# thangvubk/SoftGroup

Hardware: AMD Instinct MI355X
Metric: scans/sec ScanNet-v2-like inference (softgroup_scannet.yaml, full forward_test) (higher is better)
Workload: dtype f32

## Files before the change

softgroup_amd/csrc/common.h:

```cpp
#pragma once
#include <hip/hip_runtime.h>
#include <stdint.h>
#include <stdio.h>

#include "../../include/softgroup_hip.h"

namespace sg {

constexpr int kWave = 64;

void set_error(const char *fmt, ...);
int32_t *pinned_words();

inline hipStream_t as_stream(sg_stream_t s) { return reinterpret_cast<hipStream_t>(s); }

inline int check_launch(const char *what) {
  hipError_t e = hipGetLastError();
  if (e != hipSuccess) {
    set_error("%s: %s", what, hipGetErrorString(e));
    return SG_ERR_LAUNCH;
  }
  return SG_OK;
}

// ... 55 lines not shown
  v += dpp_or_zero<0x142, 0xa>(v);
  v += dpp_or_zero<0x143, 0xc>(v);
  return v;
}
__device__ __forceinline__ int wave_sum(int v) {
  return __builtin_amdgcn_readlane(wave_incl_scan(v), 63);
}
__device__ __forceinline__ int wave_max(int v) {
#pragma unroll
  for (int o = 32; o > 0; o >>= 1) v = max(v, __shfl_xor(v, o, 64));
  return v;
}

constexpr int kFillMax = 16;
struct FillList {
  uint32_t *p[kFillMax];
  size_t words[kFillMax];
  uint32_t pattern[kFillMax];
  int n = 0;
  void add(void *ptr, size_t bytes, int byte) {
    if (bytes == 0 || ptr == nullptr || n >= kFillMax) return;
    p[n] = static_cast<uint32_t *>(ptr);
    words[n] = bytes / 4;
    pattern[n] = 0x01010101u * static_cast<uint32_t>(byte & 0xff);
    ++n;
  }
};
static __global__ void __launch_bounds__(256) fill_many_kernel(FillList f) {
  const int r = blockIdx.y;
  uint32_t *p = f.p[r];
  const size_t w = f.words[r];
  const uint32_t v = f.pattern[r];
  const size_t head = (16 - (reinterpret_cast<uintptr_t>(p) & 15)) / 4 % 4;
  const size_t h = head < w ? head : w;
  const size_t quads = (w - h) / 4;
  uint4 *q = reinterpret_cast<uint4 *>(p + h);
  const uint4 vv = make_uint4(v, v, v, v);
  for (size_t i = blockIdx.x * 256ull + threadIdx.x; i < quads; i += gridDim.x * 256ull) q[i] = vv;
  if (blockIdx.x == 0) {
    if (threadIdx.x < h) p[threadIdx.x] = v;
    const size_t t0 = h + quads * 4;
    if (threadIdx.x < w - t0) p[t0 + threadIdx.x] = v;
  }
}
inline void fill_many(const FillList &f, hipStream_t stream) {
  if (f.n == 0) return;
  size_t mx = 0;
  for (int i = 0; i < f.n; ++i) mx = f.words[i] > mx ? f.words[i] : mx;
  const int gx = grid_for(static_cast<int64_t>(mx / 4 + 1), 256, 1024);
  fill_many_kernel<<<dim3(gx, f.n), 256, 0, stream>>>(f);
}

extern thread_local int t_conv_arith;
void conv_chain_begin(hipStream_t stream);
bool conv_chain_recording();
int conv_chain_end();
void conv_chain_abort();
int conv_chain_concat(const float *a, const float *b, int64_t rows, int ca, int cb, const float *scale,
                      const float *shift, float *out, float *out_act);
int conv_chain_bn_relu(const float *x, const float *scale, const float *shift, int64_t rows, int c, float *out);
int conv_chain_check_abort(const char *who);
int conv_gather_rows(const void *in, int num_in_rows, const int32_t *nbr, int M_out, int K, int Cin, int Cout,
                     const float *w_k8, const float *post_scale, const float *post_shift, const void *residual,
                     const float *act_scale, const float *act_shift, void *out_act, const int32_t *order,
                     const uint32_t *tile_mask, const int32_t *nbr_tiles, void *out, void *ws, size_t ws_bytes,
                     sg_stream_t stream, int in16, int out16, int res16);
int spconv_wgrad_layout(const void *in, int in_bf16, const void *g_out, int g_bf16, const int32_t *nbr_t, int M_out,
                        int K, int Cin, int Cout, float *dw, int out_oki, void *ws, size_t ws_bytes,
                        sg_stream_t stream);
struct PackJob {
  const float *w;
  float *out;
  int cout, kvol, cin, mode;
};
int spconv_pack_weights(const PackJob *jobs, int n, sg_stream_t stream);
size_t octree_stash_bytes(int n);
int octree_ballquery_count_stash(const float *points, const float *boxes, const int32_t *pt_inds,
                                 const int32_t *pt_start_len, int n, float radius, int32_t *start_len, int32_t *stash,
                                 hipStream_t stream);
int octree_ballquery_fill_stash(const float *points, const float *boxes, const int32_t *pt_inds,
                                const int32_t *pt_start_len, int n, float radius, const int32_t *start_len,
                                const int32_t *stash, int32_t *idx, hipStream_t stream);
void conv_release_stream(int dev, hipStream_t stream);
void unet_release_stream(int dev, hipStream_t stream);
void scan_release_stream(int dev, hipStream_t stream);
void bfs_release_stream(int dev, hipStream_t stream);
constexpr int kBfsGiantMin = 16384;
struct BfsDefer {
  bool deferred = false;
  hipStream_t side = nullptr;
};
void bfs_emit_defer(BfsDefer *d);
int bfs_emit_join(const BfsDefer &d, hipStream_t stream);
int bfs_label_max_kept(const void *ws);
int bfs_count_kept_members(const void *ws, size_t ws_bytes, int n, int64_t n_edges, const int32_t *l2p, int n_pts,
                           const float *thr_dev, int32_t *out, hipStream_t stream);

}
```

softgroup_amd/csrc/spconv_conv.hip:

```cpp
#include <stdlib.h>

#include <atomic>
#include <cstdio>
#include <map>
#include <mutex>
#include <utility>
#include <vector>

#include "common.h"

namespace sg {

typedef float f32x16 __attribute__((ext_vector_type(16)));
typedef float f4 __attribute__((ext_vector_type(4)));
typedef float f2 __attribute__((ext_vector_type(2)));
typedef __bf16 bf16x8 __attribute__((ext_vector_type(8)));
typedef __bf16 bf16x2 __attribute__((ext_vector_type(2)));

__device__ __forceinline__ void split3(const float (&x)[8], bf16x8 &h, bf16x8 &m, bf16x8 &l) {
#pragma unroll
  for (int j = 0; j < 4; ++j) {
    const f2 v = {x[2 * j], x[2 * j + 1]};
    const bf16x2 hh = __builtin_convertvector(v, bf16x2);
    const f2 r = v - __builtin_convertvector(hh, f2);
// ... 18 lines not shown
__device__ __forceinline__ uint16_t bf16_rne(float x) {
  const uint32_t u = __builtin_bit_cast(uint32_t, x);
  return static_cast<uint16_t>((u + 0x7fffu + ((u >> 16) & 1u)) >> 16);
}
__device__ __forceinline__ float bf16_f32(uint16_t b) {
  return __builtin_bit_cast(float, static_cast<uint32_t>(b) << 16);
}

#ifndef SG_WHATIF
#define SG_WHATIF 0
#endif

constexpr int kTileRows = 32;
constexpr int kWavesPerWg = 4;
constexpr int kCk = 16;
constexpr int kMaxK = 27;
constexpr int kTicketStride = 32;
constexpr unsigned kOob = 0x80000000u;

__device__ __forceinline__ void lds_dma_b128(const void *gsrc, unsigned lds_dst) {
  unsigned keep;
  asm volatile("s_mov_b32 %0, m0\n\ts_mov_b32 m0, %2\n\ts_nop 0\n\tglobal_load_lds_dwordx4 %1, off\n\t"
               "s_mov_b32 m0, %0"
               : "=&s"(keep) : "v"(gsrc), "s"(lds_dst) : "memory");
}
__device__ __forceinline__ void lds_dma_b32(const void *gsrc, unsigned lds_dst) {
  unsigned keep;
  asm volatile("s_mov_b32 %0, m0\n\ts_mov_b32 m0, %2\n\ts_nop 0\n\tglobal_load_lds_dword %1, off\n\t"
               "s_mov_b32 m0, %0"
               : "=&s"(keep) : "v"(gsrc), "s"(lds_dst) : "memory");
}

struct ConvArgs {
  const float *in;
  const int32_t *nbr;
  const float *w;
  const float *post_scale;
  const float *post_shift;
  const float *residual;
  const float *act_scale;
  const float *act_shift;
  float *out_act;
  const int32_t *order;
  const uint32_t *tile_mask;
  const int32_t *nbr_tiles;
  float *out;
  int M_out, K, Cin, Cout;
  int col_units;
  int blocks_per_unit;
  int ksplit;
  int k_per_split;
  int num_units;
  unsigned magic_upt, magic_cu, magic_nsl;
  int out16, res16;
  int dyn_rounds;
  unsigned *queue;
  unsigned long long *trace;
  unsigned *done;
  float *out_final;
};

template <int NBW, bool VEC>
__global__ void __launch_bounds__(256) gather_conv_tile_kernel(ConvArgs p) {
  extern __shared__ __attribute__((aligned(16))) char smem_raw[];
  const int wave = threadIdx.x >> 6, lane = threadIdx.x & 63;
  int32_t *nbr_lds = reinterpret_cast<int32_t *>(smem_raw) + wave * kTileRows * kMaxK;
  const int cin_pad = (p.Cin + kCk - 1) / kCk * kCk;
  const int c8 = (p.Cin + 7) / 8;

  const int num_tiles = (p.M_out + kTileRows - 1) / kTileRows;
  const int units_per_tile = p.col_units * p.ksplit;
  const long long unit = static_cast<long long>(blockIdx.x) * kWavesPerWg + wave;
  const bool valid = unit < static_cast<long long>(num_tiles) * units_per_tile;
  int tile = valid ? static_cast<int>(unit / units_per_tile) : 0;
  const int sub = valid ? static_cast<int>(unit % units_per_tile) : 0;
  const int cu = sub % p.col_units, ks = sub / p.col_units;
  const int nb0 = cu * p.blocks_per_unit;
  const int nbw = valid ? min(p.blocks_per_unit, (p.Cout + 31) / 32 - nb0) : 0;
  const int k_lo = ks * p.k_per_split, k_hi = min(p.K, k_lo + p.k_per_split);

  const int arow = lane & 31, ahalf = lane >> 5;
  int my_row = -1;
  if (valid) {
    const int pos = tile * kTileRows + arow;
    if (p.order) my_row = p.order[pos];
    else if (pos < p.M_out) my_row = pos;
  }
  if (valid) {
    for (int e = lane; e < kTileRows * p.K; e += 64) {
      const int r = e / p.K, k = e - r * p.K;
      const int row = __shfl(my_row, r, 64);
      nbr_lds[r * kMaxK + k] = row >= 0 ? p.nbr[static_cast<long long>(row) * p.K + k] : -1;
    }
  }
  __syncthreads();
  if (!valid) return;

  uint32_t mask = p.tile_mask ? p.tile_mask[tile] : 0xffffffffu;
  mask &= (k_hi >= 32 ? 0xffffffffu : ((1u << k_hi) - 1u)) & ~((1u << k_lo) - 1u);

  f32x16 acc[NBW];
#pragma unroll
  for (int n = 0; n < NBW; ++n)
#pragma unroll
    for (int r = 0; r < 16; ++r) acc[n][r] = 0.f;

// ... 256 lines not shown
      }
      const int s_w = planes_at + (k * c8 + s * 4) * p.Cout * 16;
#pragma unroll
      for (int n = 0; n < NBW; ++n)
#pragma unroll
        for (int sl = 0; sl < 2; ++sl)
#pragma unroll
          for (int pl = 0; pl < NPL; ++pl) {
            if ((SG_WHATIF & 1) && pl > 0) { S.b[n][sl * NPL + pl] = S.b[n][sl * NPL]; continue; }
            S.b[n][sl * NPL + pl] = __builtin_bit_cast(f4, __builtin_amdgcn_raw_buffer_load_b128(
                                                             rs_w, c.v_w + n * 512,
                                                             s_w + sl * (2 * p.Cout * 16) + pl * plane_bytes, 0));
          }
      return;
    }
    const int src = c.meta[nbr_base + k];
    const unsigned v_a = src >= 0 ? static_cast<unsigned>(src * p.Cin + ahalf * HC) * 4u : kOob;
    const int s_a = s * (CK * 4);
#pragma unroll
    for (int q = 0; q < NQ; ++q)
      S.a[q] = __builtin_bit_cast(f4, __builtin_amdgcn_raw_buffer_load_b128(rs_in, v_a + q * 16, s_a, AUX));
    if constexpr (SPLIT) {
      const int s_w = planes_at + (k * c8 + s * 2) * p.Cout * 16;
#pragma unroll
      for (int n = 0; n < NBW; ++n)
#pragma unroll
        for (int pl = 0; pl < NPL; ++pl)
          S.b[n][pl] = __builtin_bit_cast(f4, __builtin_amdgcn_raw_buffer_load_b128(
                                                  rs_w, c.v_w + n * 512, s_w + pl * plane_bytes, 0));
    } else {
      const int s_w = (k * c8 + s * (CK / 8)) * p.Cout * 32;
#pragma unroll
      for (int n = 0; n < NBW; ++n)
#pragma unroll
        for (int q = 0; q < NQ; ++q)
          S.b[n][q] = __builtin_bit_cast(f4, __builtin_amdgcn_raw_buffer_load_b128(
                                                 rs_w, c.v_w + n * 1024 + (q & 1) * 16,
                                                 s_w + (q >> 1) * (p.Cout * 32), 0));
    }
  };

  auto advance = [&](const Ctx &c, int &k, int &s) {
    if (++s == n_slices) {
      s = 0;
      const uint32_t rest = c.wg_mask & ~((2u << k) - 1u);
      k = rest ? __builtin_ctz(rest) : k;
    }
  };

  auto setup = [&](const Unit &d, int buf, Ctx &c) {
    c.ks = d.ks;
    c.pair = d.tile * p.col_units + d.cu;
    c.meta = meta_lds + buf * kMetaInts;
    uint32_t m = static_cast<uint32_t>(c.meta[kMaskAt]);
    if (!final_out) {
      const int k_lo = d.ks * p.k_per_split, k_hi = min(p.K, k_lo + p.k_per_split);
      m &= ((1u << k_hi) - 1u) & ~((1u << k_lo) - 1u);
    }
    m = __builtin_amdgcn_readfirstlane(m);
    c.wg_mask = m;
    c.col = d.cu * (32 * NBW) + arow;
    c.col_ok = c.col < p.Cout;
    const int colc = min(c.col, p.Cout - 1);
    c.v_w = SPLIT ? (ahalf * p.Cout + colc) * 16 : (ahalf * (HC / 8) * p.Cout + colc) * 32;
    const int items = __builtin_popcount(m) * n_slices;
    const int per = (items + WV - 1) >> WV_SHIFT;
    const int begin = min(items, wave * per);
    c.rem = min(items, begin + per) - begin;
    int rank = udiv(begin, p.magic_nsl);
    c.s = begin - rank * n_slices;
    uint32_t mm = m;
    for (; rank > 0; --rank) mm &= mm - 1u;
    c.k = mm ? __builtin_ctz(mm) : 0;
    load(c, c.k, c.s, S[0]);
    c.kp = c.k;
    c.sp = c.s;
#pragma unroll
    for (int i = 1; i < DEPTH - 1; ++i) {
      if (i < c.rem) advance(c, c.kp, c.sp);
      load(c, c.kp, c.sp, S[i]);
    }
    int row4[RR];
#pragma unroll
    for (int rr = 0; rr < RR; ++rr) {
      const int reg = wave * RR + rr;
      row4[rr] = c.meta[kRowsAt + (reg & 3) + 8 * (reg >> 2) + 4 * ahalf];
    }
#pragma unroll
    for (int rr = 0; rr < RR; ++rr) {
      const unsigned off = (row4[rr] >= 0 && c.col_ok)
                               ? static_cast<unsigned>(row4[rr] * p.Cout + c.col) * 4u : kOob;
      c.o_off[rr] = off;
#pragma unroll
      for (int n = 0; n < NBW; ++n)
        resv[n][rr] = ld_row(rs_res, off, n, res16);
    }
#pragma unroll
    for (int n = 0; n < NBW; ++n) {
      c.ps[n] = c.pb[n] = c.as[n] = c.ab[n] = 0.f;
      if (post) {
        c.ps[n] = p.post_scale[colc + 32 * n];
        c.pb[n] = p.post_shift[colc + 32 * n];
      }
      if (act) {
        c.as[n] = p.act_scale[colc + 32 * n];
        c.ab[n] = p.act_shift[colc + 32 * n];
      }
    }
  };

  f32x16 acc[NBW];
  auto compute = [&](Slice &S) {
    if constexpr (R16) {
#pragma unroll
      for (int q = 0; q < 4; ++q) {
        const int r = 8 * q + (lane >> 3);
        tr_lds[r * 8 + ((lane & 7) ^ ((r >> 1) & 7))] = S.a[q];
      }
      f4 fr[4];
#pragma unroll
      for (int sl = 0; sl < 4; ++sl) fr[sl] = tr_lds[arow * 8 + ((sl * 2 + ahalf) ^ ((arow >> 1) & 7))];
// ... 204 lines not shown

    float v[NBW][RR], va[NBW][RR];
    unsigned o_off[RR];
    {
      float part[NBW][RR][WV];
#pragma unroll
      for (int n = 0; n < NBW; ++n)
#pragma unroll
        for (int rr = 0; rr < RR; ++rr) {
          const int reg = wave * RR + rr;
#pragma unroll
          for (int w = 0; w < WV; ++w) part[n][rr][w] = red[((w * NBW + n) * 16 + reg) * 64 + lane];
        }
#pragma unroll
      for (int rr = 0; rr < RR; ++rr) {
#pragma unroll
        for (int n = 0; n < NBW; ++n) {
          float t = part[n][rr][0];
#pragma unroll
          for (int w = 1; w < WV; ++w) t += part[n][rr][w];
          t += resv[n][rr];
          if (post) t = fmaxf(fmaf(t, c.ps[n], c.pb[n]), 0.f);
          v[n][rr] = t;
          va[n][rr] = fmaxf(fmaf(t, c.as[n], c.ab[n]), 0.f);
        }
        o_off[rr] = c.o_off[rr];
      }
    }
    const unsigned o_base = final_out ? 0u : static_cast<unsigned>(c.ks) * out_bytes;
    const int rem_done = c.rem;
    const int pair_done = c.pair, col_done = c.col;
    setup(dn, has_next ? (buf ^ 1) : buf, c);
    mark(4);
    if (combine) {
#pragma unroll
      for (int rr = 0; rr < RR; ++rr)
#pragma unroll
        for (int n = 0; n < NBW; ++n)
          __builtin_amdgcn_raw_buffer_store_b32(__builtin_bit_cast(unsigned, v[n][rr]), rs_out, o_off[rr],
                                                o_base + n * 128, 16);
    } else {
#pragma unroll
    for (int rr = 0; rr < RR; ++rr)
#pragma unroll
      for (int n = 0; n < NBW; ++n) st_row(v[n][rr], rs_out, o_off[rr], o_base, n, out16 && final_out);
    }
    if (act) {
#pragma unroll
      for (int rr = 0; rr < RR; ++rr)
#pragma unroll
        for (int n = 0; n < NBW; ++n) st_row(va[n][rr], rs_act, o_off[rr], 0u, n, out16);
    }
    if (combine) {
      asm volatile("s_waitcnt vmcnt(0)" ::: "memory");
      barrier();
      if (wave == 0 && lane == 0) {
        const unsigned arrived = __hip_atomic_fetch_add(p.done + pair_done, 1u, __ATOMIC_RELAXED,
                                                        __HIP_MEMORY_SCOPE_AGENT);
        ctl[3] = arrived == static_cast<unsigned>(p.ksplit - 1);
      }
      barrier();
      if (__builtin_amdgcn_readfirstlane(ctl[3]) != 0) {
        const int colc = min(col_done, p.Cout - 1);
        float ps[NBW], pb[NBW], as[NBW], ab[NBW];
#pragma unroll
        for (int n = 0; n < NBW; ++n) {
          ps[n] = pb[n] = as[n] = ab[n] = 0.f;
          if (p.post_scale) { ps[n] = p.post_scale[colc + 32 * n]; pb[n] = p.post_shift[colc + 32 * n]; }
          if (c_act) { as[n] = p.act_scale[colc + 32 * n]; ab[n] = p.act_shift[colc + 32 * n]; }
        }
        auto part = [&](int ks, int rr, int n) {
          return __builtin_bit_cast(float, __builtin_amdgcn_raw_buffer_load_b32(
                                               rs_out, o_off[rr], static_cast<unsigned>(ks) * out_bytes + n * 128, 16));
        };
        float t[NBW][RR];
#pragma unroll
        for (int rr = 0; rr < RR; ++rr)
#pragma unroll
          for (int n = 0; n < NBW; ++n) t[n][rr] = part(0, rr, n);
        int ks = 1;
        for (; ks + 3 < p.ksplit; ks += 4) {
          float q[4][NBW][RR];
#pragma unroll
          for (int j = 0; j < 4; ++j)
#pragma unroll
            for (int rr = 0; rr < RR; ++rr)
#pragma unroll
              for (int n = 0; n < NBW; ++n) q[j][n][rr] = part(ks + j, rr, n);
#pragma unroll
          for (int j = 0; j < 4; ++j)
#pragma unroll
            for (int rr = 0; rr < RR; ++rr)
#pragma unroll
              for (int n = 0; n < NBW; ++n) t[n][rr] += q[j][n][rr];
        }
        for (; ks < p.ksplit; ++ks) {
          float q[NBW][RR];
#pragma unroll
          for (int rr = 0; rr < RR; ++rr)
#pragma unroll
            for (int n = 0; n < NBW; ++n) q[n][rr] = part(ks, rr, n);
#pragma unroll
          for (int rr = 0; rr < RR; ++rr)
#pragma unroll
            for (int n = 0; n < NBW; ++n) t[n][rr] += q[n][rr];
        }
        float res[NBW][RR];
#pragma unroll
        for (int rr = 0; rr < RR; ++rr)
#pragma unroll
          for (int n = 0; n < NBW; ++n)
            res[n][rr] = ld_row(rs_cres, o_off[rr], n, res16);
#pragma unroll
        for (int rr = 0; rr < RR; ++rr)
#pragma unroll
          for (int n = 0; n < NBW; ++n) {
            float x = t[n][rr] + res[n][rr];
            if (p.post_scale) x = fmaxf(fmaf(x, ps[n], pb[n]), 0.f);
            st_row(x, rs_cout, o_off[rr], 0u, n, out16);
            st_row(fmaxf(fmaf(x, as[n], ab[n]), 0.f), rs_cact, o_off[rr], 0u, n, out16);
          }
      }
    }
    mark(5);
    if constexpr (TRACE) {
      if (lane == 0 && p.trace && wave < kWavesPerWg) {
        unsigned long long *t = p.trace + (static_cast<long long>(u) * kWavesPerWg + wave) * 8;
        for (int i = 0; i < 6; ++i) t[i] = stamp[i];
        unsigned hw, xcc;
        asm volatile("s_getreg_b32 %0, hwreg(HW_REG_HW_ID)" : "=s"(hw));
        asm volatile("s_getreg_b32 %0, hwreg(HW_REG_XCC_ID)" : "=s"(xcc));
        t[6] = static_cast<unsigned long long>(blockIdx.x);
        t[7] = (static_cast<unsigned long long>(rem_done) << 48) | (static_cast<unsigned long long>(xcc & 0xf) << 32) | hw;
      }
    }
    if (!has_next) break;
    u = un;
    ++round;
    buf ^= 1;
  }
}

template <int CK, int DEPTH, int TRACE, int WPE, int NBW = 1, int SPLIT = 0, int WV = 4, int AT = 0, int R16 = 0>
__global__ void __launch_bounds__(64 * WV, WPE) gather_conv_persistent_kernel(ConvArgs p, unsigned in_bytes,
                                                                             unsigned w_bytes) {
  conv_layer_body<CK, DEPTH, TRACE, NBW, SPLIT, WV, AT, 0, R16>(p, in_bytes, w_bytes);
}

struct ChainStep {
  const float *in, *w, *post_scale, *post_shift, *residual, *act_scale, *act_shift;
  float *out_act;
  const int32_t *order;
  const uint32_t *tile_mask;
  const int32_t *nbr_tiles;
  float *out;
  unsigned *done;
  float *out_final;
  int M_out, K, Cin, Cout, col_units, ksplit, k_per_split, num_units;
  unsigned magic_upt, magic_cu, magic_nsl, in_bytes, w_bytes;
  int kind;
  int pad_[2];
};
constexpr int kChainMax = 22;
struct ChainArgs {
  ChainStep s[kChainMax];
  unsigned *bar;
  unsigned *abort_host;
  unsigned long long *trace;
  int n;
};
static_assert(sizeof(ChainArgs) <= 4096, "the step list must fit the kernel-argument segment");
constexpr int kChainWV = 8;
constexpr int kChainBarWords = 18 * 32;
constexpr unsigned long long kChainTimeout = 200000000ull;

__device__ __forceinline__ bool chain_barrier(unsigned *bar, unsigned epoch, unsigned *abort_host, int *flag_lds,
                                              unsigned long long *stamp) {
  asm volatile("s_waitcnt vmcnt(0)" ::: "memory");
  __syncthreads();
  if (threadIdx.x == 0) {
    if (stamp) stamp[2] = __builtin_amdgcn_s_memrealtime();
    const unsigned x = blockIdx.x & 7, nx = (gridDim.x + 7u - x) >> 3;
    int ok = 1;
    const unsigned old = __hip_atomic_fetch_add(bar + x * 32, 1u, __ATOMIC_RELAXED, __HIP_MEMORY_SCOPE_AGENT);
    if (old == nx * epoch - 1u) {
      const unsigned groups = gridDim.x < 8u ? gridDim.x : 8u;
      const unsigned o2 = __hip_atomic_fetch_add(bar + 8 * 32, 1u, __ATOMIC_RELAXED, __HIP_MEMORY_SCOPE_AGENT);
      if (o2 == groups * epoch - 1u)
        for (unsigned j = 0; j < groups; ++j)
          __hip_atomic_store(bar + (9 + j) * 32, epoch, __ATOMIC_RELAXED, __HIP_MEMORY_SCOPE_AGENT);
    }
    const unsigned long long t0 = __builtin_amdgcn_s_memrealtime();
    unsigned spins = 0;
    while (__hip_atomic_load(bar + (9 + x) * 32, __ATOMIC_RELAXED, __HIP_MEMORY_SCOPE_AGENT) < epoch) {
      __builtin_amdgcn_s_sleep(2);
      if ((++spins & 255u) == 0u) {
        if (__hip_atomic_load(bar + 17 * 32, __ATOMIC_RELAXED, __HIP_MEMORY_SCOPE_AGENT) != 0u) { ok = 0; break; }
        if (__builtin_amdgcn_s_memrealtime() - t0 > kChainTimeout) {
          __hip_atomic_store(bar + 17 * 32, 1u, __ATOMIC_RELAXED, __HIP_MEMORY_SCOPE_AGENT);
          __hip_atomic_store(abort_host, 1u, __ATOMIC_RELAXED, __HIP_MEMORY_SCOPE_SYSTEM);
          ok = 0;
          break;
        }
      }
    }
    *flag_lds = ok;
    if (stamp) stamp[3] = __builtin_amdgcn_s_memrealtime();
  }
  __syncthreads();
  return *flag_lds != 0;
}

__device__ __forceinline__ void chain_elementwise(const ChainStep &s) {
  const int ca4 = s.Cin >> 2, cb4 = s.kind == 1 ? s.Cout >> 2 : 0, c4 = ca4 + cb4;
  const unsigned total = static_cast<unsigned>(s.M_out) * c4;
  const __amdgpu_buffer_rsrc_t ra = __builtin_amdgcn_make_buffer_rsrc(
      const_cast<float *>(s.in), 0, static_cast<unsigned>(s.M_out) * ca4 * 16u, 0x00020000);
  const __amdgpu_buffer_rsrc_t rb = __builtin_amdgcn_make_buffer_rsrc(
      const_cast<float *>(cb4 ? s.residual : s.in), 0, static_cast<unsigned>(s.M_out) * cb4 * 16u, 0x00020000);
  const __amdgpu_buffer_rsrc_t ro = __builtin_amdgcn_make_buffer_rsrc(s.out, 0, total * 16u, 0x00020000);
  const __amdgpu_buffer_rsrc_t roa = __builtin_amdgcn_make_buffer_rsrc(
      s.out_act ? s.out_act : s.out, 0, s.out_act ? total * 16u : 0u, 0x00020000);
  const float *sc = s.kind == 1 ? s.act_scale : s.post_scale, *sh = s.kind == 1 ? s.act_shift : s.post_shift;
  for (unsigned t = blockIdx.x * blockDim.x + threadIdx.x; t < total; t += gridDim.x * blockDim.x) {
    const unsigned r = t / c4, c = t - r * c4;
    f4 v;
    if (c < static_cast<unsigned>(ca4))
      v = __builtin_bit_cast(f4, __builtin_amdgcn_raw_buffer_load_b128(ra, (r * ca4 + c) * 16u, 0, 16));
    else
      v = __builtin_bit_cast(f4, __builtin_amdgcn_raw_buffer_load_b128(rb, (r * cb4 + (c - ca4)) * 16u, 0, 16));
    f4 a = v;
    if (sc != nullptr) {
      const f4 k = *reinterpret_cast<const f4 *>(sc + 4 * c), h = *reinterpret_cast<const f4 *>(sh + 4 * c);
#pragma unroll
      for (int j = 0; j < 4; ++j) a[j] = fmaxf(fmaf(v[j], k[j], h[j]), 0.f);
    }
    if (s.kind == 1) {
      __builtin_amdgcn_raw_buffer_store_b128(__builtin_bit_cast(__attribute__((ext_vector_type(4))) unsigned, v), ro, t * 16u, 0, 16);
      __builtin_amdgcn_raw_buffer_store_b128(__builtin_bit_cast(__attribute__((ext_vector_type(4))) unsigned, a), roa, t * 16u, 0, 16);
    } else {
      __builtin_amdgcn_raw_buffer_store_b128(__builtin_bit_cast(__attribute__((ext_vector_type(4))) unsigned, a), ro, t * 16u, 0, 16);
    }
  }
}

template <int SPLIT>
__global__ void __launch_bounds__(64 * kChainWV, 1) conv_chain_kernel(ChainArgs a) {
  extern __shared__ __attribute__((aligned(16))) char smem_raw[];
  int *flag_lds = reinterpret_cast<int *>(smem_raw) + kChainWV * 16 * 64 + 2 * kMetaInts + 2;
#pragma nounroll
  for (int i = 0; i < a.n; ++i) {
    const ChainStep &s = a.s[i];
    unsigned long long *stamp = a.trace ? a.trace + (static_cast<size_t>(i) * gridDim.x + blockIdx.x) * 4 : nullptr;
    if (stamp && threadIdx.x == 0) stamp[0] = __builtin_amdgcn_s_memrealtime();
    if (s.kind == 0) {
      ConvArgs p;
      p.in = s.in; p.nbr = nullptr; p.w = s.w; p.post_scale = s.post_scale; p.post_shift = s.post_shift;
      p.residual = s.residual; p.act_scale = s.act_scale; p.act_shift = s.act_shift; p.out_act = s.out_act;
      p.order = s.order; p.tile_mask = s.tile_mask; p.nbr_tiles = s.nbr_tiles; p.out = s.out;
      p.M_out = s.M_out; p.K = s.K; p.Cin = s.Cin; p.Cout = s.Cout;
      p.col_units = s.col_units; p.blocks_per_unit = 1; p.ksplit = s.ksplit; p.k_per_split = s.k_per_split;
      p.num_units = s.num_units;
      p.magic_upt = s.magic_upt; p.magic_cu = s.magic_cu; p.magic_nsl = s.magic_nsl;
      p.queue = nullptr; p.dyn_rounds = 2; p.out16 = 0; p.res16 = 0; p.trace = nullptr; p.done = s.done; p.out_final = s.out_final;
      conv_layer_body<32, 2, 0, 1, SPLIT, kChainWV, 1, 1>(p, s.in_bytes, s.w_bytes);
    } else {
      chain_elementwise(s);
    }
    if (stamp && threadIdx.x == 0) stamp[1] = __builtin_amdgcn_s_memrealtime();
    if (i + 1 < a.n && !chain_barrier(a.bar, static_cast<unsigned>(i + 1), a.abort_host, flag_lds, stamp)) return;
  }
}

__global__ void __launch_bounds__(256) conv_reduce_kernel(const float4 *__restrict__ partial,
                                                         const float4 *__restrict__ residual,
                                                         const float *__restrict__ post_scale,
                                                         const float *__restrict__ post_shift,
                                                         const float *__restrict__ act_scale,
                                                         const float *__restrict__ act_shift,
                                                         float4 *__restrict__ out_act,
                                                         int ksplit, long long n4, int cout4,
                                                         float4 *__restrict__ out) {
  for (long long t = blockIdx.x * 256LL + threadIdx.x; t < n4; t += gridDim.x * 256LL) {
    float4 a = partial[t];
    for (int s = 1; s < ksplit; ++s) {
      const float4 b = partial[s * n4 + t];
      a.x += b.x; a.y += b.y; a.z += b.z; a.w += b.w;
    }
    if (residual) {
      const float4 r = residual[t];
      a.x += r.x; a.y += r.y; a.z += r.z; a.w += r.w;
    }
    if (post_scale) {
      const int c = static_cast<int>(t % cout4) * 4;
      a.x = fmaxf(fmaf(a.x, post_scale[c], post_shift[c]), 0.f);
      a.y = fmaxf(fmaf(a.y, post_scale[c + 1], post_shift[c + 1]), 0.f);
      a.z = fmaxf(fmaf(a.z, post_scale[c + 2], post_shift[c + 2]), 0.f);
      a.w = fmaxf(fmaf(a.w, post_scale[c + 3], post_shift[c + 3]), 0.f);
    }
    out[t] = a;
    if (out_act) {
      const int c = static_cast<int>(t % cout4) * 4;
      a.x = fmaxf(fmaf(a.x, act_scale[c], act_shift[c]), 0.f);
      a.y = fmaxf(fmaf(a.y, act_scale[c + 1], act_shift[c + 1]), 0.f);
      a.z = fmaxf(fmaf(a.z, act_scale[c + 2], act_shift[c + 2]), 0.f);
      a.w = fmaxf(fmaf(a.w, act_scale[c + 3], act_shift[c + 3]), 0.f);
      out_act[t] = a;
    }
  }
}

__global__ void __launch_bounds__(256) gather_conv_scalar_kernel(
    const float *__restrict__ in, const int32_t *__restrict__ nbr, int M_out, int K, int Cin,
    int Cout, const float *__restrict__ w_k8, const float *__restrict__ post_scale,
    const float *__restrict__ post_shift, const float *__restrict__ residual,
    const float *__restrict__ act_scale, const float *__restrict__ act_shift,
// ... 193 lines not shown
  if (t != g_ticket_pools.end()) {
    if (t->second.dev) hipFree(t->second.dev);
    g_ticket_pools.erase(t);
  }
}

static unsigned *take_tickets(hipStream_t stream) {
  int dev = 0;
  hipGetDevice(&dev);
  std::lock_guard<std::mutex> lock(g_ticket_mu);
  TicketPool &tp = g_ticket_pools[{dev, stream}];
  if (tp.dev == nullptr) {
    if (hipMalloc(&tp.dev, kTicketBlocks * kTicketBlockBytes) != hipSuccess) return nullptr;
    tp.next = kTicketBlocks;
  }
  if (tp.next == kTicketBlocks) {
    hipMemsetAsync(tp.dev, 0, kTicketBlocks * kTicketBlockBytes, stream);
    tp.next = 0;
  }
  return tp.dev + (8 * kTicketStride) * tp.next++;
}


struct ChainRec {
  int mode = 0;
  bool b16 = false;
  bool arith_set = false;
  int conv_steps = 0;
  hipStream_t stream = nullptr;
  ChainArgs args;
};
static thread_local ChainRec t_chain;
static std::atomic<int> g_chain_override{-1};
static std::atomic<long long> g_chain_launches{0}, g_chain_steps{0};
static std::mutex g_chain_mu;
static std::map<int, hipEvent_t> g_chain_last;
static std::map<std::pair<int, hipStream_t>, hipEvent_t> g_chain_events;
static std::map<int, unsigned *> g_chain_abort;

static void chain_release_stream(int dev, hipStream_t stream) {
  std::lock_guard<std::mutex> lock(g_chain_mu);
  auto it = g_chain_events.find({dev, stream});
  if (it == g_chain_events.end()) return;
  auto last = g_chain_last.find(dev);
  if (last != g_chain_last.end() && last->second == it->second) last->second = nullptr;
  if (it->second) hipEventDestroy(it->second);
  g_chain_events.erase(it);
}

static bool chain_enabled() {
  static const int env = getenv("SG_CONV_CHAIN") ? atoi(getenv("SG_CONV_CHAIN")) : 0;
  const int ov = g_chain_override.load(std::memory_order_relaxed);
  return (ov >= 0 ? ov : env) != 0;
}

int conv_chain_check_abort(const char *who) {
  int dev = 0;
  hipGetDevice(&dev);
  std::lock_guard<std::mutex> lock(g_chain_mu);
  auto it = g_chain_abort.find(dev);
  if (it != g_chain_abort.end() && *static_cast<volatile unsigned *>(it->second) != 0u) {
    *static_cast<volatile unsigned *>(it->second) = 0u;
    set_error("%s: a grid barrier of an earlier multi-layer conv launch timed out (its workgroups were not "
              "co-resident: another process on this GPU?); that forward's results are invalid. "
              "SG_CONV_CHAIN=0 launches the layers one by one", who);
    return SG_ERR_LAUNCH;
  }
  return SG_OK;
}

static int chain_flush() {
  ChainRec &c = t_chain;
  if (c.args.n == 0) return SG_OK;
  int dev = 0;
  hipGetDevice(&dev);
  static int num_cu = 0;
  static std::once_flag once;
  std::call_once(once, [&] {
    hipDeviceGetAttribute(&num_cu, hipDeviceAttributeMultiprocessorCount, dev);
    if (num_cu <= 0) num_cu = 256;
  });
  c.args.bar = take_done(c.stream, kChainBarWords);
  if (c.args.bar == nullptr) {
    set_error("conv chain: no barrier block");
    return SG_ERR_LAUNCH;
  }
  const size_t lds = static_cast<size_t>(kChainWV) * 16 * 64 * sizeof(float) + 2 * kMetaInts * sizeof(int32_t) + 16 +
                     static_cast<size_t>(kChainWV) * 4096;
  static const int grid_env = getenv("SG_CHAIN_GRID") ? atoi(getenv("SG_CHAIN_GRID")) : 0;
  static const bool serial = !(getenv("SG_CHAIN_SERIAL") && atoi(getenv("SG_CHAIN_SERIAL")) == 0);
  int grid = num_cu >= 8 ? num_cu - num_cu % 8 : num_cu;
  if (grid_env >= 8 && grid_env < grid) grid = grid_env - grid_env % 8;
  const bool prof = g_conv_prof.enabled && c.conv_steps > 0;
  {
    std::lock_guard<std::mutex> lock(g_chain_mu);
    unsigned *&ab = g_chain_abort[dev];
    if (ab == nullptr) {
      if (hipHostMalloc(reinterpret_cast<void **>(&ab), 64, hipHostMallocMapped) != hipSuccess) {
        ab = nullptr;
        set_error("conv chain: pinned allocation failed");
        return SG_ERR_LAUNCH;
      }
      *ab = 0u;
    }
    c.args.abort_host = ab;
    hipEvent_t &mine = g_chain_events[{dev, c.stream}];
// ... 144 lines not shown
    if (num_cu <= 0) num_cu = 256;
    auto prepare = [](SplitVariant &v) {
      v.lds = static_cast<size_t>(v.wv) * v.nbw * 16 * 64 * sizeof(float) + 2 * kMetaInts * sizeof(int32_t) + 16 +
              (v.at ? static_cast<size_t>(v.wv) * 4096 : 0);
      int o = 0;
      hipOccupancyMaxActiveBlocksPerMultiprocessor(&o, v.fn, 64 * v.wv, v.lds);
      v.occ = o < 1 ? 1 : o;
      o = 0;
      hipOccupancyMaxActiveBlocksPerMultiprocessor(&o, v.fn_b16, 64 * v.wv, v.lds);
      v.occ_b16 = o < 1 ? 1 : o;
      o = 0;
      if (v.fn_r16) hipOccupancyMaxActiveBlocksPerMultiprocessor(&o, v.fn_r16, 64 * v.wv, v.lds);
      v.occ_r16 = o < 1 ? 1 : o;
    };
    for (SplitVariant &v : g_split_variants) prepare(v);
  });
  static const int nbw_env = getenv("SG_CONV_NBW") ? atoi(getenv("SG_CONV_NBW")) : 2;
  static const int wv_env = getenv("SG_CONV_WV") ? atoi(getenv("SG_CONV_WV")) : 0;
  static const float min_rounds = getenv("SG_CONV_ROUNDS") ? atof(getenv("SG_CONV_ROUNDS")) : 2.5f;
  static const int at_env = getenv("SG_CONV_AT") ? atoi(getenv("SG_CONV_AT")) : 1;
  const int NB = (a.Cout + 31) / 32;
  const unsigned long long row_bytes = (in16 ? 2ull : 4ull) * a.Cin;
  const unsigned absent_at = static_cast<unsigned>((0xFFFFFFull * row_bytes) & 0xFFFFFFFFull);
  const int use_at = ((at_env != 0 || in16) && a.Cin % 32 == 0 && in_bytes / static_cast<long long>(row_bytes) < (1LL << 24) - 1 &&
                      static_cast<long long>(absent_at) >= in_bytes) ? 1 : 0;
  if (in16 && (!use_at || !b16)) {
    set_error("sg_unet_forward(bf16 rows): a layer with %d input channels / %lld input bytes cannot take the line-wise bf16 gather",
              a.Cin, in_bytes);
    return SG_ERR_ARG;
  }
  int pick = -1;
  static const int w2_max = getenv("SG_CONV_W2_MAX") ? atoi(getenv("SG_CONV_W2_MAX")) : 108;
  static const int w2_nbw = getenv("SG_CONV_W2_NBW") ? atoi(getenv("SG_CONV_W2_NBW")) : 2;
  static const float w2_rounds = getenv("SG_CONV_W2_ROUNDS") ? atof(getenv("SG_CONV_W2_ROUNDS")) : 1.5f;
  const bool use_w2 = wv_env == 2 || (wv_env == 0 && a.K * (a.Cin / 32) <= w2_max);
  for (int i = 0; i < kSplitVariants; ++i) {
    const SplitVariant &v = g_split_variants[i];
    if (v.at != use_at) continue;
    if (v.wv == 2 && (!use_w2 || a.ksplit > 1 || v.nbw > w2_nbw)) continue;
    if (a.ksplit > 1) {
      if (v.nbw == 1 && v.wv == 4) { pick = i; break; }
      continue;
    }
    pick = i;
    if (v.nbw == 2 && (a.Cout % 64 != 0 || nbw_env < 2)) continue;
    if (wv_env && v.wv != wv_env) continue;
    const long long units = static_cast<long long>(num_tiles) * (NB / v.nbw);
    if (wv_env || units >= static_cast<long long>((v.wv == 2 ? w2_rounds : min_rounds) * num_cu * (in16 ? v.occ_r16 : b16 ? v.occ_b16 : v.occ))) {
      pick = i;
      break;
    }
  }
  const bool chain_layer = t_chain.mode != 0 && use_at != 0;
  if (chain_layer) {
    for (int i = 0; i < kSplitVariants; ++i)
      if (g_split_variants[i].at == 1 && g_split_variants[i].nbw == 1 && g_split_variants[i].wv == kChainWV) pick = i;
  }
  const SplitVariant &v = g_split_variants[pick];
  a.col_units = NB / v.nbw;
  a.blocks_per_unit = v.nbw;
  const long long units = static_cast<long long>(num_tiles) * a.col_units * a.ksplit;
  a.num_units = static_cast<int>(units);
  auto magic = [](unsigned d) { return d <= 1 ? 0u : static_cast<unsigned>((1ULL << 32) / d) + 1u; };
  a.magic_upt = magic(static_cast<unsigned>(a.col_units * a.ksplit));
  a.magic_cu = magic(static_cast<unsigned>(a.col_units));
  a.magic_nsl = magic(static_cast<unsigned>(in16 ? (a.Cin + 63) / 64 : a.Cin / v.ck));
  if (t_chain.mode == 2) {
    if (chain_layer && !in16 && !a.out16 && !a.res16 && (a.ksplit == 1 || a.done != nullptr) && stream == t_chain.stream) {
      ChainStep st = {};
      st.kind = 0;
      st.in = a.in; st.w = a.w; st.post_scale = a.post_scale; st.post_shift = a.post_shift; st.residual = a.residual;
      st.act_scale = a.act_scale; st.act_shift = a.act_shift; st.out_act = a.out_act; st.order = a.order;
      st.tile_mask = a.tile_mask; st.nbr_tiles = a.nbr_tiles; st.out = a.out; st.done = a.done; st.out_final = a.out_final;
      st.M_out = a.M_out; st.K = a.K; st.Cin = a.Cin; st.Cout = a.Cout; st.col_units = a.col_units;
      st.ksplit = a.ksplit; st.k_per_split = a.k_per_split; st.num_units = a.num_units;
      st.magic_upt = a.magic_upt; st.magic_cu = a.magic_cu; st.magic_nsl = a.magic_nsl;
      st.in_bytes = static_cast<unsigned>(in_bytes); st.w_bytes = static_cast<unsigned>(w_bytes);
      return chain_push(st, b16, a.K > 1);
    }
    const int rc = chain_flush();
    if (rc != SG_OK) return rc;
  }
  static const bool dyn_env = getenv("SG_CONV_STATIC") && atoi(getenv("SG_CONV_STATIC")) == 0;
  static const int dyn_rounds_env = getenv("SG_CONV_DYN_ROUNDS") ? atoi(getenv("SG_CONV_DYN_ROUNDS")) : 2;
  a.queue = dyn_env ? take_tickets(stream) : nullptr;
  a.dyn_rounds = dyn_rounds_env == 1 ? 1 : 2;
  long long g = static_cast<long long>(num_cu) * (in16 ? v.occ_r16 : b16 ? v.occ_b16 : v.occ);
  if (g >= 8) g -= g % 8;
  if (units < g) g = units >= 8 ? (units + 7) / 8 * 8 : units;
  const unsigned ib = static_cast<unsigned>(in_bytes), wb = static_cast<unsigned>(w_bytes);
  if (in16) {
    v.fn_r16<<<static_cast<int>(g), 64 * v.wv, v.lds, stream>>>(a, ib, wb);
    return check_launch("sg_spconv_gather_conv(bf16 rows)");
  }
  if (b16) {
    v.fn_b16<<<static_cast<int>(g), 64 * v.wv, v.lds, stream>>>(a, ib, wb);
    return check_launch("sg_spconv_gather_conv_f32(bf16 operands)");
  }
  static const char *trace_env = getenv("SG_CONV_TRACE");
  if (trace_env) {
    const size_t nb = static_cast<size_t>(units) * kWavesPerWg * 8 * sizeof(unsigned long long);
    unsigned long long *dbuf = nullptr;
    hipMalloc(&dbuf, nb);
    hipMemsetAsync(dbuf, 0, nb, stream);
    a.trace = dbuf;
    v.fn_trace<<<static_cast<int>(g), 64 * v.wv, v.lds, stream>>>(a, ib, wb);
    hipStreamSynchronize(stream);
    std::vector<unsigned long long> h(nb / 8);
    hipMemcpy(h.data(), dbuf, nb, hipMemcpyDeviceToHost);
    hipFree(dbuf);
    if (FILE *f = fopen(trace_env, "ab")) {
      long long hdr[8] = {a.M_out, a.K, a.Cin, a.Cout, units, a.col_units, v.wv, g};
      fwrite(hdr, 8, 8, f);
      fwrite(h.data(), 8, h.size(), f);
      fclose(f);
    }
  } else {
    v.fn<<<static_cast<int>(g), 64 * v.wv, v.lds, stream>>>(a, ib, wb);
  }
  return check_launch("sg_spconv_gather_conv_f32(split)");
}


}

using namespace sg;

extern "C" {

// ... 135 lines not shown
                          static_cast<long long>(num_tiles) * kTileRows * K * 4 < (1LL << 31) &&
                          order != nullptr && tile_mask != nullptr && nbr_tiles != nullptr &&
                          reinterpret_cast<uintptr_t>(nbr_tiles) % 16 == 0;
  static const int split_env = getenv("SG_CONV_SPLIT") ? atoi(getenv("SG_CONV_SPLIT")) : 1;
  static const int split_min_cin = getenv("SG_CONV_SPLIT_MIN_CIN") ? atoi(getenv("SG_CONV_SPLIT_MIN_CIN")) : 16;
  const int arith_ov = t_conv_arith >= 0 ? t_conv_arith : g_arith_override.load(std::memory_order_relaxed);
  const int split_on = arith_ov >= 0 ? arith_ov : split_env;
  const bool split = persistent && split_on != 0 && Cin >= split_min_cin;
  static const int target_env = getenv("SG_CONV_TARGET") ? atoi(getenv("SG_CONV_TARGET")) : 0;
  const int target = target_env > 0 ? target_env : split ? 1024 : 2048;
  const int waves_per_unit = persistent ? kWavesPerWg : 1;
  int bpu = 1;
  if (!persistent) {
    bpu = NB < 4 ? NB : 4;
    while (bpu > 1 && static_cast<long long>(num_tiles) * ((NB + bpu - 1) / bpu) < target) --bpu;
  }
  const int col_units = (NB + bpu - 1) / bpu;
  int ksplit = 1;
  const long long waves = static_cast<long long>(num_tiles) * col_units * waves_per_unit;
  if (waves < target / 2) {
    const long long want = (target / 2 + waves - 1) / waves;
    ksplit = static_cast<int>(want < K ? want : K);
    const size_t need = static_cast<size_t>(ksplit) * M_out * Cout * sizeof(float);
    if (ksplit > 1 && (ws == nullptr || ws_bytes < need)) ksplit = 1;
  }
  const int k_per_split = (K + ksplit - 1) / ksplit;
  ksplit = (K + k_per_split - 1) / k_per_split;

  ConvArgs a;
  a.in = in; a.nbr = nbr; a.w = w_k8; a.post_scale = post_scale; a.post_shift = post_shift;
  a.residual = residual; a.act_scale = act_scale; a.act_shift = act_shift; a.out_act = out_act;
  a.order = order; a.tile_mask = tile_mask; a.nbr_tiles = nbr_tiles;
  a.out = ksplit > 1 ? static_cast<float *>(ws) : out;
  a.M_out = M_out; a.K = K; a.Cin = Cin; a.Cout = Cout;
  a.col_units = col_units; a.blocks_per_unit = bpu; a.ksplit = ksplit; a.k_per_split = k_per_split;
  a.trace = nullptr;
  a.queue = nullptr;
  a.dyn_rounds = 2;
  a.out16 = out16;
  a.res16 = res16;
  static const int combine_env = getenv("SG_CONV_COMBINE") ? atoi(getenv("SG_CONV_COMBINE")) : 1;
  a.done = nullptr;
  a.out_final = out;
  const int combine_ov = g_combine_override.load(std::memory_order_relaxed);
  if ((combine_ov >= 0 ? combine_ov : combine_env) != 0 && persistent && ksplit > 1 &&
      static_cast<long long>(num_tiles) * col_units <= kDoneCounters)
    a.done = take_done(stream, static_cast<size_t>(num_tiles) * col_units);
  const long long units = static_cast<long long>(num_tiles) * col_units * ksplit;
  a.num_units = static_cast<int>(units);
  auto magic = [](unsigned d) { return d <= 1 ? 0u : static_cast<unsigned>((1ULL << 32) / d) + 1u; };
  a.magic_upt = magic(static_cast<unsigned>(col_units * ksplit));
  a.magic_cu = magic(static_cast<unsigned>(col_units));
  a.magic_nsl = 0;

  if (!split && t_chain.mode == 2) {
    const int rc = chain_flush();
    if (rc != SG_OK) return rc;
  }
  if (in16 || out16 || res16) {
    SG_REQUIRE(split && split_on == 2, "sg_unet_forward(bf16 rows): layer K=%d Cin=%d Cout=%d does not run on the bf16-operand "
               "persistent kernel", K, Cin, Cout);
    SG_REQUIRE(ksplit == 1 || a.done != nullptr, "sg_unet_forward(bf16 rows): an offset-split layer needs the in-launch combine");
  }
  if (split) {
    const int rc = launch_persistent_split(a, num_tiles, in_bytes_ll, w_bytes_ll, stream, split_on == 2, in16 != 0);
    if (rc != SG_OK) return rc;
    if (t_chain.mode == 2 && t_chain.args.n > 0) return SG_OK;
  } else if (persistent) {
    const size_t lds = static_cast<size_t>(kWavesPerWg) * 16 * 64 * sizeof(float) +
                       2 * kMetaInts * sizeof(int32_t) + 16;
    constexpr int kSliceCh = 16;
    static int num_cu = 0, occ = 0;
    static std::once_flag once;
    std::call_once(once, [&] {
      int dev = 0;
      hipGetDevice(&dev);
      hipDeviceGetAttribute(&num_cu, hipDeviceAttributeMultiprocessorCount, dev);
      if (num_cu <= 0) num_cu = 256;
      hipOccupancyMaxActiveBlocksPerMultiprocessor(&occ, gather_conv_persistent_kernel<kSliceCh, 2, 0, 5>, 256, lds);
      if (occ < 1) occ = 1;
    });
    a.magic_nsl = magic(static_cast<unsigned>(Cin / kSliceCh));
    static const bool dyn_env = getenv("SG_CONV_STATIC") && atoi(getenv("SG_CONV_STATIC")) == 0;
    a.queue = dyn_env ? take_tickets(stream) : nullptr;
    a.dyn_rounds = 2;
    long long g = static_cast<long long>(num_cu) * occ;
    if (g >= 8) g -= g % 8;
    if (units < g) g = units >= 8 ? (units + 7) / 8 * 8 : units;
    const unsigned ib_ = static_cast<unsigned>(in_bytes_ll), wb_ = static_cast<unsigned>(w_bytes_ll);
    static const char *trace_env = getenv("SG_CONV_TRACE");
    if (trace_env) {
      const size_t nb = static_cast<size_t>(units) * kWavesPerWg * 8 * sizeof(unsigned long long);
      unsigned long long *dbuf = nullptr;
      hipMalloc(&dbuf, nb);
      hipMemsetAsync(dbuf, 0, nb, stream);
      a.trace = dbuf;
      gather_conv_persistent_kernel<kSliceCh, 2, 1, 5><<<static_cast<int>(g), 256, lds, stream>>>(a, ib_, wb_);
      hipStreamSynchronize(stream);
      std::vector<unsigned long long> h(nb / 8);
      hipMemcpy(h.data(), dbuf, nb, hipMemcpyDeviceToHost);
      hipFree(dbuf);
      if (FILE *f = fopen(trace_env, "ab")) {
        long long hdr[8] = {M_out, K, Cin, Cout, units, col_units, ksplit, g};
        fwrite(hdr, 8, 8, f);
        fwrite(h.data(), 8, h.size(), f);
        fclose(f);
// ... 49 lines not shown
```

softgroup_amd/csrc/unet_exec.hip:

```cpp
#include <map>
#include <mutex>
#include <utility>
#include <vector>

#include <stdlib.h>

#include "common.h"
#include "radix_sort.h"
#include "unet_common.h"

namespace sg {

__global__ void __launch_bounds__(256) batch_max_kernel(const int32_t *__restrict__ indices, int M,
                                                       int32_t *__restrict__ bmax) {
  int m = 0;
  for (int i = blockIdx.x * 256 + threadIdx.x; i < M; i += gridDim.x * 256) m = max(m, indices[4 * i]);
#pragma unroll
  for (int o = 32; o > 0; o >>= 1) m = max(m, __shfl_xor(m, o, 64));
  if ((threadIdx.x & 63) == 0 && m > 0) atomicMax(bmax, m);
}
__device__ __forceinline__ uint64_t spread3(uint32_t v) {
  uint64_t x = v & 0x1fffffu;
  x = (x | (x << 32)) & 0x1f00000000ffffull;
  x = (x | (x << 16)) & 0x1f0000ff0000ffull;
// ... 246 lines not shown
      Plan &P = li[l].ident;
      P.nbr = ord; P.order = ord; P.nbr_tiles = ord; P.tile_mask = tm;
      P.rows = li[l].rows; P.kvol = 1;
    }
    ident_plan_kernel<<<dim3(grid_for(num_rows, 256), L - 1), 256, 0, istream>>>(segs);
  }
#undef SG_IALLOC
  if (own_istream && (hipEventRecord(st.ev_index, istream) != hipSuccess ||
                      hipStreamWaitEvent(as_stream(stream), st.ev_index, 0) != hipSuccess)) {
    set_error("%s: event record/wait failed", who);
    return SG_ERR_LAUNCH;
  }
  *used = ix.off;
  *lock = std::move(guard);
  return SG_OK;
}

__global__ void __launch_bounds__(256) pad_channels_kernel(const float *__restrict__ in, int64_t rows, int cin,
                                                          int cpad, const int32_t *__restrict__ perm,
                                                          float *__restrict__ out) {
  const int64_t total = rows * cpad;
  for (int64_t t = blockIdx.x * 256LL + threadIdx.x; t < total; t += gridDim.x * 256LL) {
    const int64_t r = t / cpad;
    const int c = static_cast<int>(t - r * cpad);
    const int64_t src = perm ? perm[r] : r;
    out[t] = c < cin ? in[src * cin + c] : 0.f;
  }
}

#define SG_ALLOC(var, T, count)                                                        \
  T *var = ar.take<T>(count);                                                          \
  if (var == nullptr) {                                                                \
    set_error("sg_unet_forward: arena too small (%zu bytes, need more than %zu)", ar.cap, ar.off); \
    return SG_ERR_WORKSPACE;                                                           \
  }

thread_local void (*t_unet_conv_hook)(void *) = nullptr;
thread_local void *t_unet_conv_ctx = nullptr;

struct Exec {
  const sg_unet_desc *d;
  Arena ar;
  sg_stream_t stream;
  const LevelIdx *idx;
  const int32_t *perm = nullptr;

  Exec(const sg_unet_desc *desc, void *arena, size_t bytes, sg_stream_t s, const LevelIdx *li)
      : d(desc), ar(arena, bytes), stream(s), idx(li) {}

  bool r16 = false;
  size_t fsz(size_t n) const { return r16 ? (n + 1) / 2 : n; }
  bool chain_open = false;
  bool chain_from(int l) const {
    static const int max_rows = getenv("SG_CONV_CHAIN_ROWS") ? atoi(getenv("SG_CONV_CHAIN_ROWS")) : 6144;
    if (r16 || chain_open || idx[l].rows > max_rows || idx[l].rows <= 0) return false;
    for (int k = l; k < d->n_levels; ++k)
      if (d->levels[k].planes % 32 != 0) return false;
    return true;
  }
  struct ChainScope {
    Exec &e;
    bool on;
    ChainScope(Exec &ex, bool open) : e(ex), on(open) {
      if (on) {
        conv_chain_begin(as_stream(e.stream));
        e.chain_open = true;
      }
    }
    int close() {
      if (!on) return SG_OK;
      on = false;
      e.chain_open = false;
      return conv_chain_end();
    }
    ~ChainScope() {
      if (on) {
        conv_chain_abort();
        e.chain_open = false;
      }
    }
  };

  struct Act {
    const float *scale = nullptr, *shift = nullptr;
    float *out = nullptr;
  };

  int conv(const float *in, int in_rows, const Plan &p, int cin, int cout, const float *w,
           const float *post_s, const float *post_b, const float *residual, const Act &act, float *out,
           bool in_f32 = false, bool out_f32 = false) {
    if (p.rows == 0) return SG_OK;
    const size_t m = ar.mark();
    const size_t nb = sg_spconv_conv_workspace_bytes(p.rows, cout);
    void *ws = nullptr;
    if (nb > 256) {
      ws = ar.take<char>(nb);
    }
    const int rc = !r16 ? sg_spconv_gather_conv_f32(in, in_rows, p.nbr, p.rows, p.kvol, cin, cout, w, post_s,
                                                    post_b, residual, act.scale, act.shift, act.out, p.order,
                                                    p.tile_mask, p.nbr_tiles, out, ws, ws ? nb : 0, stream)
                        : conv_gather_rows(in, in_rows, p.nbr, p.rows, p.kvol, cin, cout, w, post_s, post_b, residual,
                                           act.scale, act.shift, act.out, p.order, p.tile_mask, p.nbr_tiles, out, ws,
                                           ws ? nb : 0, stream, in_f32 ? 0 : 1, out_f32 ? 0 : 1, 1);
    ar.release(m);
    return rc;
  }

  int block(const sg_unet_block &b, const float *x, const float *xa, int rows, const Plan &subm,
// ... 270 lines not shown
```

Before: 419.4.

## Balance offset-split work by item count and use chain kernel variant for small layers

Changes the offset-split partition in the persistent conv kernel: instead of masking each split to a fixed range of kernel offsets (which leaves splits uneven when the tile mask is sparse), work items (offset×slice) are divided evenly across splits with a magic-number divide. The post-scale/act and residual loads in the in-launch combine are hoisted before the barrier so their latency overlaps the wait. Small non-bf16 layers now pick the chain-tuned split variant even when chaining is off, and chain_from checks that chaining is enabled before opening a scope. This risks changing the summation grouping of partial sums and adds register pressure from the hoisted loads.

```diff
diff --git a/softgroup_amd/csrc/common.h b/softgroup_amd/csrc/common.h
--- a/softgroup_amd/csrc/common.h
+++ b/softgroup_amd/csrc/common.h
@@ -131,6 +131,8 @@
 }
 
 extern thread_local int t_conv_arith;
+bool conv_chain_enabled();
+int conv_chain_max_rows();
 void conv_chain_begin(hipStream_t stream);
 bool conv_chain_recording();
 int conv_chain_end();
diff --git a/softgroup_amd/csrc/spconv_conv.hip b/softgroup_amd/csrc/spconv_conv.hip
--- a/softgroup_amd/csrc/spconv_conv.hip
+++ b/softgroup_amd/csrc/spconv_conv.hip
@@ -94,6 +94,7 @@
   int k_per_split;
   int num_units;
   unsigned magic_upt, magic_cu, magic_nsl;
+  unsigned magic_ks;
   int out16, res16;
   int dyn_rounds;
   unsigned *queue;
@@ -456,21 +457,21 @@
     c.ks = d.ks;
     c.pair = d.tile * p.col_units + d.cu;
     c.meta = meta_lds + buf * kMetaInts;
-    uint32_t m = static_cast<uint32_t>(c.meta[kMaskAt]);
-    if (!final_out) {
-      const int k_lo = d.ks * p.k_per_split, k_hi = min(p.K, k_lo + p.k_per_split);
-      m &= ((1u << k_hi) - 1u) & ~((1u << k_lo) - 1u);
-    }
-    m = __builtin_amdgcn_readfirstlane(m);
+    const uint32_t m = __builtin_amdgcn_readfirstlane(static_cast<uint32_t>(c.meta[kMaskAt]));
     c.wg_mask = m;
     c.col = d.cu * (32 * NBW) + arow;
     c.col_ok = c.col < p.Cout;
     const int colc = min(c.col, p.Cout - 1);
     c.v_w = SPLIT ? (ahalf * p.Cout + colc) * 16 : (ahalf * (HC / 8) * p.Cout + colc) * 32;
-    const int items = __builtin_popcount(m) * n_slices;
+    int first = 0, items = __builtin_popcount(m) * n_slices;
+    if (!final_out) {
+      first = udiv(static_cast<unsigned>(d.ks * items), p.magic_ks);
+      items = static_cast<int>(udiv(static_cast<unsigned>((d.ks + 1) * items), p.magic_ks)) - first;
+    }
     const int per = (items + WV - 1) >> WV_SHIFT;
-    const int begin = min(items, wave * per);
-    c.rem = min(items, begin + per) - begin;
+    const int mine = min(items, wave * per);
+    c.rem = min(items, mine + per) - mine;
+    const int begin = first + mine;
     int rank = udiv(begin, p.magic_nsl);
     c.s = begin - rank * n_slices;
     uint32_t mm = m;
@@ -781,6 +782,20 @@
         for (int n = 0; n < NBW; ++n) st_row(va[n][rr], rs_act, o_off[rr], 0u, n, out16);
     }
     if (combine) {
+      const int colc = min(col_done, p.Cout - 1);
+      float ps[NBW], pb[NBW], as[NBW], ab[NBW];
+#pragma unroll
+      for (int n = 0; n < NBW; ++n) {
+        ps[n] = pb[n] = as[n] = ab[n] = 0.f;
+        if (p.post_scale) { ps[n] = p.post_scale[colc + 32 * n]; pb[n] = p.post_shift[colc + 32 * n]; }
+        if (c_act) { as[n] = p.act_scale[colc + 32 * n]; ab[n] = p.act_shift[colc + 32 * n]; }
+      }
+      float res[NBW][RR];
+#pragma unroll
+      for (int rr = 0; rr < RR; ++rr)
+#pragma unroll
+        for (int n = 0; n < NBW; ++n)
+          res[n][rr] = ld_row(rs_cres, o_off[rr], n, res16);
       asm volatile("s_waitcnt vmcnt(0)" ::: "memory");
       barrier();
       if (wave == 0 && lane == 0) {
@@ -790,14 +805,6 @@
       }
       barrier();
       if (__builtin_amdgcn_readfirstlane(ctl[3]) != 0) {
-        const int colc = min(col_done, p.Cout - 1);
-        float ps[NBW], pb[NBW], as[NBW], ab[NBW];
-#pragma unroll
-        for (int n = 0; n < NBW; ++n) {
-          ps[n] = pb[n] = as[n] = ab[n] = 0.f;
-          if (p.post_scale) { ps[n] = p.post_scale[colc + 32 * n]; pb[n] = p.post_shift[colc + 32 * n]; }
-          if (c_act) { as[n] = p.act_scale[colc + 32 * n]; ab[n] = p.act_shift[colc + 32 * n]; }
-        }
         auto part = [&](int ks, int rr, int n) {
           return __builtin_bit_cast(float, __builtin_amdgcn_raw_buffer_load_b32(
                                                rs_out, o_off[rr], static_cast<unsigned>(ks) * out_bytes + n * 128, 16));
@@ -834,12 +841,6 @@
 #pragma unroll
             for (int n = 0; n < NBW; ++n) t[n][rr] += q[n][rr];
         }
-        float res[NBW][RR];
-#pragma unroll
-        for (int rr = 0; rr < RR; ++rr)
-#pragma unroll
-          for (int n = 0; n < NBW; ++n)
-            res[n][rr] = ld_row(rs_cres, o_off[rr], n, res16);
 #pragma unroll
         for (int rr = 0; rr < RR; ++rr)
 #pragma unroll
@@ -888,7 +889,8 @@
   int M_out, K, Cin, Cout, col_units, ksplit, k_per_split, num_units;
   unsigned magic_upt, magic_cu, magic_nsl, in_bytes, w_bytes;
   int kind;
-  int pad_[2];
+  unsigned magic_ks;
+  int pad_;
 };
 constexpr int kChainMax = 22;
 struct ChainArgs {
@@ -990,7 +992,7 @@
       p.M_out = s.M_out; p.K = s.K; p.Cin = s.Cin; p.Cout = s.Cout;
       p.col_units = s.col_units; p.blocks_per_unit = 1; p.ksplit = s.ksplit; p.k_per_split = s.k_per_split;
       p.num_units = s.num_units;
-      p.magic_upt = s.magic_upt; p.magic_cu = s.magic_cu; p.magic_nsl = s.magic_nsl;
+      p.magic_upt = s.magic_upt; p.magic_cu = s.magic_cu; p.magic_nsl = s.magic_nsl; p.magic_ks = s.magic_ks;
       p.queue = nullptr; p.dyn_rounds = 2; p.out16 = 0; p.res16 = 0; p.trace = nullptr; p.done = s.done; p.out_final = s.out_final;
       conv_layer_body<32, 2, 0, 1, SPLIT, kChainWV, 1, 1>(p, s.in_bytes, s.w_bytes);
     } else {
@@ -1290,6 +1292,11 @@
   static const int env = getenv("SG_CONV_CHAIN") ? atoi(getenv("SG_CONV_CHAIN")) : 0;
   const int ov = g_chain_override.load(std::memory_order_relaxed);
   return (ov >= 0 ? ov : env) != 0;
+}
+bool conv_chain_enabled() { return chain_enabled(); }
+int conv_chain_max_rows() {
+  static const int max_rows = getenv("SG_CONV_CHAIN_ROWS") ? atoi(getenv("SG_CONV_CHAIN_ROWS")) : 6144;
+  return max_rows;
 }
 
 int conv_chain_check_abort(const char *who) {
@@ -1540,7 +1547,8 @@
     }
   }
   const bool chain_layer = t_chain.mode != 0 && use_at != 0;
-  if (chain_layer) {
+  const bool small_layer = use_at != 0 && !in16 && !a.out16 && !a.res16 && a.M_out <= conv_chain_max_rows();
+  if (chain_layer || small_layer) {
     for (int i = 0; i < kSplitVariants; ++i)
       if (g_split_variants[i].at == 1 && g_split_variants[i].nbw == 1 && g_split_variants[i].wv == kChainWV) pick = i;
   }
@@ -1562,7 +1570,7 @@
       st.tile_mask = a.tile_mask; st.nbr_tiles = a.nbr_tiles; st.out = a.out; st.done = a.done; st.out_final = a.out_final;
       st.M_out = a.M_out; st.K = a.K; st.Cin = a.Cin; st.Cout = a.Cout; st.col_units = a.col_units;
       st.ksplit = a.ksplit; st.k_per_split = a.k_per_split; st.num_units = a.num_units;
-      st.magic_upt = a.magic_upt; st.magic_cu = a.magic_cu; st.magic_nsl = a.magic_nsl;
+      st.magic_upt = a.magic_upt; st.magic_cu = a.magic_cu; st.magic_nsl = a.magic_nsl; st.magic_ks = a.magic_ks;
       st.in_bytes = static_cast<unsigned>(in_bytes); st.w_bytes = static_cast<unsigned>(w_bytes);
       return chain_push(st, b16, a.K > 1);
     }
@@ -1804,6 +1812,7 @@
   a.magic_upt = magic(static_cast<unsigned>(col_units * ksplit));
   a.magic_cu = magic(static_cast<unsigned>(col_units));
   a.magic_nsl = 0;
+  a.magic_ks = magic(static_cast<unsigned>(ksplit));
 
   if (!split && t_chain.mode == 2) {
     const int rc = chain_flush();
diff --git a/softgroup_amd/csrc/unet_exec.hip b/softgroup_amd/csrc/unet_exec.hip
--- a/softgroup_amd/csrc/unet_exec.hip
+++ b/softgroup_amd/csrc/unet_exec.hip
@@ -322,8 +322,8 @@
   size_t fsz(size_t n) const { return r16 ? (n + 1) / 2 : n; }
   bool chain_open = false;
   bool chain_from(int l) const {
-    static const int max_rows = getenv("SG_CONV_CHAIN_ROWS") ? atoi(getenv("SG_CONV_CHAIN_ROWS")) : 6144;
-    if (r16 || chain_open || idx[l].rows > max_rows || idx[l].rows <= 0) return false;
+    if (!conv_chain_enabled() || r16 || chain_open || idx[l].rows > conv_chain_max_rows() || idx[l].rows <= 0)
+      return false;
     for (int k = l; k < d->n_levels; ++k)
       if (d->levels[k].planes % 32 != 0) return false;
     return true;
```

New measurement: 414.5, median of 2. No clear change (-1.2%).
